# Lynne-Zheng-Linfang/HS-Pose

Hardware: AMD Instinct MI355X
Metric: point-clouds/sec (N=1028) HS-layer fwd+bwd (higher is better)
Workload: dtype f32; 1 GPU; HS stack (FaceRecon backbone -> feat) fwd+bwd, B=16/GPU N=1028 fp32, train-mode BN, random-init weights (BASELINE configs[1] shape); global_batch=16, points=1028, parallelism=dp1, hipgraph=True, split_graph=False, grad_exchange=none

## Files before the change

### hs_pose_amd/csrc/rfconv.hip

```cpp
#include "common.h"
#include "folds.h"
#include <stdlib.h>
#include <atomic>
#include <type_traits>

namespace hsp {

#define RF_THREADS 256

__device__ __forceinline__ void normalise_dirs(float4& d0, float4& d1, float4& d2) {
#define RF_NRM(X)                                                                                    \
    {                                                                                                \
        const float n2 = norm2_chain(d0.X, d1.X, d2.X);                                              \
        const float nr = fmaxf(sqrtf(n2), 1e-12f);                     \
        d0.X = __fdiv_rn(d0.X, nr); d1.X = __fdiv_rn(d1.X, nr); d2.X = __fdiv_rn(d2.X, nr);          \
    }
    RF_NRM(x) RF_NRM(y) RF_NRM(z) RF_NRM(w)
#undef RF_NRM
}
__device__ __forceinline__ void load_dirs_normed(const float* __restrict__ dirs, int SC, int j, float4& d0,
                                                 float4& d1, float4& d2) {
    d0 = *reinterpret_cast<const float4*>(dirs + j);
    d1 = *reinterpret_cast<const float4*>(dirs + SC + j);
    d2 = *reinterpret_cast<const float4*>(dirs + 2 * SC + j);
    normalise_dirs(d0, d1, d2);
}

#ifdef RF_RELU_MAX
#define RF_RELU(X) fmaxf((X), 0.f)
#else
#define RF_RELU(X) __builtin_amdgcn_fmed3f((X), 0.f, 1.f)
#endif

struct PointIter {
    int b0, bstep, i0, istep;
    __device__ __forceinline__ PointIter(int B) {
        const int xcd = blockIdx.x % HSP_NUM_XCD;
        const int local = blockIdx.x / HSP_NUM_XCD;
        const int per_xcd = gridDim.x / HSP_NUM_XCD;
        if (B >= HSP_NUM_XCD) {
            b0 = xcd; bstep = HSP_NUM_XCD; i0 = local; istep = per_xcd;
        } else {
            b0 = xcd % B; bstep = B * HSP_NUM_XCD;
            const int share = xcd / B;
            const int nshare = (HSP_NUM_XCD - b0 + B - 1) / B;
            i0 = local + per_xcd * share; istep = per_xcd * nshare;
        }
    }
};

template <class R3>
__device__ __forceinline__ float rf_dot3(const R3 r, float d0, float d1, float d2) { return dot3_chain(r.x, r.y, r.z, d0, d1, d2); }

template <int NCH>
__device__ __forceinline__ void rf_load_dirs(const float* dirs, int SC, int tid, float4 (&d0)[NCH], float4 (&d1)[NCH],
                                             float4 (&d2)[NCH]) {
    const int nq = SC >> 2;
#pragma unroll
    for (int u = 0; u < NCH; ++u) {
        const int cq = tid + u * RF_THREADS;
        load_dirs_normed(dirs, SC, (cq < nq ? cq : 0) << 2, d0[u], d1[u], d2[u]);
    }
}

template <bool SURFACE, bool WF, typename FT, class Fetch>
__device__ __forceinline__ void rf_group_body(const float4 d0, const float4 d1, const float4 d2, const float4* sR, const int* sIdx,
                                              int k, Fetch fetch, float* smax_j, uint16_t* arg_pj, FT* fwin_pj) {
    float4 best = make_float4(-INFINITY, -INFINITY, -INFINITY, -INFINITY);
    int a0 = 0, a1 = 0, a2 = 0, a3 = 0;
    float4 wf = make_float4(1.f, 1.f, 1.f, 1.f);
#pragma unroll 4
    for (int n = 0; n < k; ++n) {
        const float4 r = sR[n];
        float4 th;
        th.x = RF_RELU(rf_dot3(r, d0.x, d1.x, d2.x));
        th.y = RF_RELU(rf_dot3(r, d0.y, d1.y, d2.y));
        th.z = RF_RELU(rf_dot3(r, d0.z, d1.z, d2.z));
        th.w = RF_RELU(rf_dot3(r, d0.w, d1.w, d2.w));
        if (!SURFACE) {
            const float4 f = fetch(n);
            th.x = mul_rn(th.x, f.x); th.y = mul_rn(th.y, f.y);
            th.z = mul_rn(th.z, f.z); th.w = mul_rn(th.w, f.w);
            if (WF) {
                if (th.x > best.x) wf.x = f.x;
                if (th.y > best.y) wf.y = f.y;
                if (th.z > best.z) wf.z = f.z;
                if (th.w > best.w) wf.w = f.w;
            }
        }
        if (th.x > best.x) { best.x = th.x; a0 = n; }
        if (th.y > best.y) { best.y = th.y; a1 = n; }
        if (th.z > best.z) { best.z = th.z; a2 = n; }
        if (th.w > best.w) { best.w = th.w; a3 = n; }
    }
    *reinterpret_cast<float4*>(smax_j) = best;
    {
        const unsigned lo = (unsigned)sIdx[a0] | ((unsigned)sIdx[a1] << 16);
        const unsigned hi = (unsigned)sIdx[a2] | ((unsigned)sIdx[a3] << 16);
        unsigned* ap = reinterpret_cast<unsigned*>(arg_pj);
        __builtin_nontemporal_store(lo, ap); __builtin_nontemporal_store(hi, ap + 1);
    }
    if (WF) Feat<FT>::st4_nt(fwin_pj, wf);
}

template <bool SURFACE, typename FT>
__device__ __forceinline__ void rf_mean_phase(const float* smax, const FT* fm, FT* out, size_t pt, int S,
                                              int C, float invS_div, int tid) {
    const int fstride = (S + 1) * C;
    for (int c = tid; c < C; c += RF_THREADS) {
        float s = smax[c];
        for (int sp = 1; sp < S; ++sp) s = add_rn(s, smax[sp * C + c]);
        float v = __fdiv_rn(s, invS_div);
        if (!SURFACE) v = add_rn(Feat<FT>::ld(fm + pt * fstride + c), v);
        Feat<FT>::st_nt(out + pt * C + c, v);
    }
}

template <bool SURFACE, int NCH, bool WF, typename FT>
__global__ __launch_bounds__(RF_THREADS) void rf_fwd_kernel(const float* __restrict__ xyz,
                                                            const int32_t* __restrict__ idx,
                                                            const float* __restrict__ dirs,
                                                            const FT* __restrict__ fm, int B, int N, int k,
                                                            int S, int C, FT* __restrict__ out,
                                                            uint16_t* __restrict__ argrow,
                                                            FT* __restrict__ fwin) {
    extern __shared__ __attribute__((aligned(16))) char smem[];
    const int SC = S * C;
    float* smax = reinterpret_cast<float*>(smem);
    float4* sR = reinterpret_cast<float4*>(smax + SC);
    int* sIdx = reinterpret_cast<int*>(sR + k);
    const int tid = threadIdx.x;
    const int nq = SC >> 2;
    const int fstride = (S + 1) * C;
    const float invS_div = (float)S;
    float4 d0[NCH], d1[NCH], d2[NCH];
    rf_load_dirs<NCH>(dirs, SC, tid, d0, d1, d2);
    const PointIter it(B);
    for (int b = it.b0; b < B; b += it.bstep) {
        const float* xb = xyz + (size_t)b * N * 3;
        for (int i = it.i0; i < N; i += it.istep) {
            const size_t pt = (size_t)b * N + i;
            __syncthreads();
            for (int t = tid; t < k; t += RF_THREADS) {
                const int m = idx[pt * k + t];
                sIdx[t] = m;
                const float3 r = unit_dir(xb[i * 3], xb[i * 3 + 1], xb[i * 3 + 2], xb[m * 3], xb[m * 3 + 1], xb[m * 3 + 2]);
                sR[t] = make_float4(r.x, r.y, r.z, 0.f);
            }
            __syncthreads();
#pragma unroll
            for (int u = 0; u < NCH; ++u) {
                const int cq = tid + u * RF_THREADS;
                if (cq < nq) {
                    const int j = cq << 2;
                    const FT* fsup = SURFACE ? nullptr : fm + (size_t)b * N * fstride + C + j;
                    auto fetch = [=](int n) { return Feat<FT>::ld4(fsup + (size_t)sIdx[n] * fstride); };
                    rf_group_body<SURFACE, WF, FT>(d0[u], d1[u], d2[u], sR, sIdx, k, fetch, smax + j, argrow + pt * SC + j,
                                                   WF ? fwin + pt * SC + j : nullptr);
                }
            }
            __syncthreads();
            rf_mean_phase<SURFACE, FT>(smax, fm, out, pt, S, C, invS_div, tid);
        }
    }
}


template <bool SURFACE, int NCH, bool WF, typename FT>
__global__ __launch_bounds__(RF_THREADS) void rf_fwd_pipe_kernel(const float* __restrict__ xyz,
                                                                 const int32_t* __restrict__ idx,
                                                                 const float* __restrict__ dirs,
                                                                 const FT* __restrict__ fm, int B, int N, int k,
                                                                 int S, int C, FT* __restrict__ out,
                                                                 uint16_t* __restrict__ argrow,
                                                                 FT* __restrict__ fwin) {
    extern __shared__ __attribute__((aligned(16))) char smem[];
    const int SC = S * C;
    float* smax2 = reinterpret_cast<float*>(smem);
    float4* sR2 = reinterpret_cast<float4*>(smax2 + 2 * SC);
    int* sIdx2 = reinterpret_cast<int*>(sR2 + 2 * k);
    unsigned* sOff2 = reinterpret_cast<unsigned*>(sIdx2 + 2 * k);
    const int tid = threadIdx.x;
    const int nq = SC >> 2;
    const int fstride = (S + 1) * C;
    const int spare0 = nq - (NCH - 1) * RF_THREADS;
    const float invS_div = (float)S;
    float4 d0[NCH], d1[NCH], d2[NCH];
    rf_load_dirs<NCH>(dirs, SC, tid, d0, d1, d2);
    const PointIter it(B);
    auto dirs_phase = [&](int b, int i, int buf) {
        const int t = tid - spare0;
        if (t >= 0 && t < k) {
            const float* xb = xyz + (size_t)b * N * 3;
            const int m = idx[((size_t)b * N + i) * k + t];
            sIdx2[buf * k + t] = m;
            sOff2[buf * k + t] = (unsigned)m * (unsigned)fstride * (unsigned)sizeof(FT);
            const float3 r = unit_dir(xb[i * 3], xb[i * 3 + 1], xb[i * 3 + 2], xb[m * 3], xb[m * 3 + 1], xb[m * 3 + 2]);
            sR2[buf * k + t] = make_float4(r.x, r.y, r.z, 0.f);
        }
    };
    int b = it.b0, i = it.i0;
    bool have = b < B && i < N;
    if (have) dirs_phase(b, i, 0);
    int cur = 0;
    bool have_prev = false;
    size_t prev_pt = 0;
    while (have) {
        int nb = b, ni = i + it.istep;
        if (ni >= N) { nb = b + it.bstep; ni = it.i0; }
        const bool have_next = nb < B;
        const size_t pt = (size_t)b * N + i;
        __syncthreads();
        if (have_prev) rf_mean_phase<SURFACE, FT>(smax2 + (cur ^ 1) * SC, fm, out, prev_pt, S, C, invS_div, tid);
        if (have_next) dirs_phase(nb, ni, cur ^ 1);
        float* smax = smax2 + cur * SC;
        const float4* sR = sR2 + cur * k;
        const int* sIdx = sIdx2 + cur * k;
        const unsigned* sOff = sOff2 + cur * k;
#pragma unroll
        for (int u = 0; u < NCH; ++u) {
            const int cq = tid + u * RF_THREADS;
            if (cq < nq) {
                const int j = cq << 2;
                const unsigned long long fbase = reinterpret_cast<unsigned long long>(SURFACE ? out : fm + (size_t)b * N * fstride);
                FT* ubase = reinterpret_cast<FT*>(((unsigned long long)__builtin_amdgcn_readfirstlane((unsigned)(fbase >> 32)) << 32) |
                                                  (unsigned)__builtin_amdgcn_readfirstlane((unsigned)fbase));
                const __amdgpu_buffer_rsrc_t frs =
                    __builtin_amdgcn_make_buffer_rsrc(ubase, 0, (int)((size_t)N * fstride * sizeof(FT)), 0x00020000);
                const unsigned voff = (unsigned)(C + j) * (unsigned)sizeof(FT);
                auto fetch = [=](int n) {
                    if constexpr (sizeof(FT) == 4) {
                        const auto v = __builtin_amdgcn_raw_buffer_load_b128(frs, (int)(voff + sOff[n]), 0, 0);
                        return make_float4(__uint_as_float(v[0]), __uint_as_float(v[1]), __uint_as_float(v[2]), __uint_as_float(v[3]));
                    } else {
                        const auto v = __builtin_amdgcn_raw_buffer_load_b64(frs, (int)(voff + sOff[n]), 0, 0);
                        return make_float4(__uint_as_float(v[0] << 16), __uint_as_float(v[0] & 0xffff0000u),
                                           __uint_as_float(v[1] << 16), __uint_as_float(v[1] & 0xffff0000u));
                    }
                };
                rf_group_body<SURFACE, WF, FT>(d0[u], d1[u], d2[u], sR, sIdx, k, fetch, smax + j,
                                               argrow + pt * SC + j, WF ? fwin + pt * SC + j : nullptr);
            }
        }
        have_prev = true; prev_pt = pt;
        cur ^= 1;
        b = nb; i = ni; have = have_next;
    }
    __syncthreads();
    if (have_prev) rf_mean_phase<SURFACE, FT>(smax2 + (cur ^ 1) * SC, fm, out, prev_pt, S, C, invS_div, tid);
}

#define RF_EB 8

template <int NCH>
__global__ __launch_bounds__(RF_THREADS) void rf_conv_bwd_csr_kernel(
    const float* __restrict__ xyz, const float* __restrict__ dirs, const float* __restrict__ fm,
    const uint16_t* __restrict__ argrow, const float* __restrict__ gout, const int32_t* __restrict__ rev_off,
    const int32_t* __restrict__ rev_edge, int B, int N, int k, int S, int C, float* __restrict__ gfm,
    float* __restrict__ ws) {
    extern __shared__ __attribute__((aligned(16))) char smem[];
    const int SC = S * C;
    float* sg = reinterpret_cast<float*>(smem);
    float4* sR = reinterpret_cast<float4*>(sg + RF_EB * C);
    int* sI = reinterpret_cast<int*>(sR + RF_EB);
    const int tid = threadIdx.x;
    const int nq = SC >> 2;
    const int fstride = (S + 1) * C;
    const float invS = 1.0f / (float)S;
    const int cq4 = C >> 2;

    float4 d0[NCH], d1[NCH], d2[NCH], gd0[NCH], gd1[NCH], gd2[NCH];
    rf_load_dirs<NCH>(dirs, SC, tid, d0, d1, d2);
#pragma unroll
    for (int u = 0; u < NCH; ++u) gd0[u] = gd1[u] = gd2[u] = make_float4(0.f, 0.f, 0.f, 0.f);
    const PointIter it(B);
    for (int b = it.b0; b < B; b += it.bstep) {
        const float* xb = xyz + (size_t)b * N * 3;
        const int32_t* offb = rev_off + (size_t)b * (N + 1);
        const int32_t* edgeb = rev_edge + (size_t)b * N * k;
        for (int m = it.i0; m < N; m += it.istep) {
            const size_t pm = (size_t)b * N + m;
            const int o0 = offb[m], o1 = offb[m + 1];
            const float mx = xb[m * 3], my = xb[m * 3 + 1], mz = xb[m * 3 + 2];
            float4 fv[NCH], acc[NCH];
#pragma unroll
            for (int u = 0; u < NCH; ++u) {
                const int cq = tid + u * RF_THREADS;
                acc[u] = make_float4(0.f, 0.f, 0.f, 0.f);
                fv[u] = cq < nq ? *reinterpret_cast<const float4*>(fm + pm * fstride + C + (cq << 2)) : acc[u];
            }
            for (int c = tid; c < C; c += RF_THREADS) gfm[pm * fstride + c] = gout[pm * C + c];
            for (int e0 = o0; e0 < o1; e0 += RF_EB) {
                const int ne = min(RF_EB, o1 - e0);
                __syncthreads();
                if (tid < ne) {
                    const int e = edgeb[e0 + tid];
                    const int i = e / k, n = e - i * k;
                    const float3 r = unit_dir(xb[i * 3], xb[i * 3 + 1], xb[i * 3 + 2], mx, my, mz);
                    sR[tid] = make_float4(r.x, r.y, r.z, __int_as_float(n));
                    sI[tid] = i;
                }
                __syncthreads();
                for (int q = tid; q < ne * cq4; q += RF_THREADS) {
                    const int t = q / cq4, c4 = q - t * cq4;
                    float4 g = *reinterpret_cast<const float4*>(gout + ((size_t)b * N + sI[t]) * C + (c4 << 2));
                    g.x *= invS; g.y *= invS; g.z *= invS; g.w *= invS;
                    *reinterpret_cast<float4*>(sg + t * C + (c4 << 2)) = g;
                }
                __syncthreads();
#pragma unroll
                for (int u = 0; u < NCH; ++u) {
                    const int cq = tid + u * RF_THREADS;
                    if (cq < nq) {
                        const int j = cq << 2;
                        const int c = j % C;
                        ushort4 am[RF_EB];
#pragma unroll
                        for (int t = 0; t < RF_EB; ++t)
                            am[t] = *reinterpret_cast<const ushort4*>(argrow + ((size_t)b * N + sI[t < ne ? t : 0]) * SC + j);
#pragma unroll
                        for (int t = 0; t < RF_EB; ++t) {
                            if (t < ne) {
                                const float4 r = sR[t];
                                const int n = m;
                                const float4 ga = *reinterpret_cast<const float4*>(sg + t * C + c);
#define RF_ONE(X)                                                                                         \
    if (am[t].X == n) {                                                                                   \
        const float z = rf_dot3(r, d0[u].X, d1[u].X, d2[u].X);                                            \
        if (z > 0.f) {                                                                                    \
            acc[u].X += ga.X * z;                                                                         \
            const float w = ga.X * fv[u].X;                                                               \
            gd0[u].X += w * r.x; gd1[u].X += w * r.y; gd2[u].X += w * r.z;                                \
// ... 318 lines not shown
    }
    __syncthreads();
    if (!SURFACE) {
        for (int q = tid; q < (r1 - r0) * G; q += RF_TILE_THREADS) {
            const int m = q / G, g4 = q - m * G;
            const int4 iv = *reinterpret_cast<const int4*>(acc + m * TC + g4 * 4);
            Feat<FT>::st4(gfm + ((size_t)b * N + r0 + m) * fstride + C + j0 + g4 * 4,
                          make_float4((float)iv.x * fx_inv, (float)iv.y * fx_inv, (float)iv.z * fx_inv, (float)iv.w * fx_inv));
        }
        if (D == 0 && j0 < C) {
            for (int q = tid; q < (r1 - r0) * G; q += RF_TILE_THREADS) {
                const int m = q / G, g4 = q - m * G;
                Feat<FT>::st4(gfm + ((size_t)b * N + r0 + m) * fstride + j0 + g4 * 4,
                              Feat<FT>::ld4(gout + ((size_t)b * N + r0 + m) * C + j0 + g4 * 4));
            }
        }
        __syncthreads();
    }
    float* red = reinterpret_cast<float*>(smem);
    float* mine = red + tid * 12;
    mine[0] = g0.x; mine[1] = g0.y; mine[2] = g0.z; mine[3] = g0.w;
    mine[4] = g1.x; mine[5] = g1.y; mine[6] = g1.z; mine[7] = g1.w;
    mine[8] = g2.x; mine[9] = g2.y; mine[10] = g2.z; mine[11] = g2.w;
    __syncthreads();
    if (tid < G * 12) {
        const int gg = tid / 12, w = tid - gg * 12;
        float sacc = 0.f;
        for (int l = 0; l < PL; ++l) sacc += red[(l * G + gg) * 12 + w];
        const int d = w >> 2, e = w & 3;
        gd_part[((size_t)(b * RS + (RS > 1 ? (int)blockIdx.z : 0)) * 3 + d) * SC + j0 + gg * 4 + e] = sacc;
    }
}

__global__ __launch_bounds__(1024) void rf_dirs_reduce_kernel(const float* __restrict__ ws, int nblk, int SC,
                                                              const float* __restrict__ dirs,
                                                              float* __restrict__ out) {
    __shared__ float red[16][3][64];
    dirs_fold_body<1024>(ws, nblk, SC, dirs, out, (int)blockIdx.x, red);
}

static int rf_bwd_grid_max(int SC) {
    long long g = (8ll << 20) / (12ll * SC);
    g &= ~7ll;
    if (g < 8) g = 8;
    if (g > 1024) g = 1024;
    return (int)g;
}

static int rf_bwd_grid(long long points, int SC) {
    const int g = persistent_blocks(points, 4), gm = rf_bwd_grid_max(SC);
    return g < gm ? g : gm;
}

}

using namespace hsp;

static int rf_check(const void* a, const void* b, const void* c, int B, int N, int k, int S, int C) {
    if (!a || !b || !c || B <= 0 || N <= 0 || k <= 0 || S <= 0 || C <= 0) return HSP_ERR_BAD_ARG;
    if (N > 65535 || (C & 3)) return HSP_ERR_UNSUPPORTED;
    return HSP_OK;
}

struct RfFwdPlan { int nch; bool pipe; size_t lds; };
static RfFwdPlan rf_fwd_plan(int k, int S, int C) {
    RfFwdPlan p{0, false, 0};
    if (k <= 0 || S <= 0 || C <= 0 || (C & 3) || (long long)S * C > 4096 || k > 16384) return p;
    const size_t lds = (size_t)(S * C + 5 * k) * 4;
    if (lds > 64 * 1024) return p;
    p.nch = ((S * C >> 2) + RF_THREADS - 1) / RF_THREADS;
    p.lds = lds;
    const int spare0 = (S * C >> 2) - (p.nch - 1) * RF_THREADS;
    const size_t lds_pipe = 2 * (size_t)(S * C + 6 * k) * 4;
    if (spare0 + k <= RF_THREADS && lds_pipe <= 64 * 1024) { p.pipe = true; p.lds = lds_pipe; }
    return p;
}

extern "C" int hsp_rf_fwd_plan(int k, int S, int C, int* pipelined) {
    const RfFwdPlan p = rf_fwd_plan(k, S, C);
    if (pipelined) *pipelined = p.pipe ? 1 : 0;
    return p.nch;
}

template <class F>
static void rf_dispatch_nch(int nch, bool wf, F launch) {
    auto with_wf = [&](auto n) {
        if (wf) launch(n, std::true_type{});
        else launch(n, std::false_type{});
    };
    switch (nch) {
        case 1: with_wf(std::integral_constant<int, 1>{}); break;
        case 2: with_wf(std::integral_constant<int, 2>{}); break;
        case 3: with_wf(std::integral_constant<int, 3>{}); break;
        default: with_wf(std::integral_constant<int, 4>{}); break;
    }
}

template <bool SURFACE, typename FT>
static int rf_fwd(const float* xyz, const int32_t* idx, const float* dirs, const FT* fm, int B, int N, int k,
                  int S, int C, FT* out, uint16_t* argrow, FT* fwin, hspStream_t stream) {
    int rc = rf_check(xyz, idx, dirs, B, N, k, S, C);
    if (rc) return rc;
    if (!out || !argrow || (!SURFACE && !fm)) return HSP_ERR_BAD_ARG;
    const RfFwdPlan plan = rf_fwd_plan(k, S, C);
    if (!plan.nch) return HSP_ERR_UNSUPPORTED;
    const long long npts = (long long)B * N;
    const int grid = persistent_blocks(npts, npts < 2048 ? 4 : npts < 8192 ? 6 : 8);
    rf_dispatch_nch(plan.nch, !SURFACE && fwin, [&](auto nch, auto wf) {
        constexpr int NCH = decltype(nch)::value;
        constexpr bool WF = !SURFACE && decltype(wf)::value;
        auto kern = plan.pipe ? rf_fwd_pipe_kernel<SURFACE, NCH, WF, FT> : rf_fwd_kernel<SURFACE, NCH, WF, FT>;
        hipLaunchKernelGGL(kern, dim3(grid), dim3(RF_THREADS), plan.lds, as_stream(stream), xyz, idx, dirs, fm, B, N, k, S, C, out,
                           argrow, fwin);
    });
    return check_launch();
}

extern "C" int hsp_rf_surface_fwd(const float* xyz, const int32_t* idx, const float* dirs_n, int B, int N, int k,
                                  int S, int K, float* out, uint16_t* argrow, hspStream_t stream) {
    return rf_fwd<true, float>(xyz, idx, dirs_n, nullptr, B, N, k, S, K, out, argrow, nullptr, stream);
}
extern "C" int hsp_rf_surface_fwd_bf16(const float* xyz, const int32_t* idx, const float* dirs_n, int B, int N, int k,
                                       int S, int K, hsp_bf16_t* out, uint16_t* argrow, hspStream_t stream) {
    return rf_fwd<true, bf16_t>(xyz, idx, dirs_n, nullptr, B, N, k, S, K, out, argrow, nullptr, stream);
}

extern "C" int hsp_rf_conv_wants_fwin(int N, int S, int C) {
    (void)N; (void)S; (void)C;
    return 1;
}

extern "C" int hsp_rf_conv_fwd(const float* xyz, const int32_t* idx, const float* dirs_n, const float* fm, int B,
                               int N, int k, int S, int C, float* out, uint16_t* argrow, float* fwin,
                               hspStream_t stream) {
    return rf_fwd<false, float>(xyz, idx, dirs_n, fm, B, N, k, S, C, out, argrow, fwin, stream);
}
extern "C" int hsp_rf_conv_fwd_bf16(const float* xyz, const int32_t* idx, const float* dirs_n, const hsp_bf16_t* fm, int B,
                                    int N, int k, int S, int C, hsp_bf16_t* out, uint16_t* argrow, hsp_bf16_t* fwin,
                                    hspStream_t stream) {
    return rf_fwd<false, bf16_t>(xyz, idx, dirs_n, fm, B, N, k, S, C, out, argrow, fwin, stream);
}
extern "C" int hsp_rf_conv_wants_fwin_bf16(int N, int S, int C) {
    return (size_t)N * (S + 1) * C * sizeof(bf16_t) >= ((size_t)3 << 20) ? 1 : 0;
}

extern "C" size_t hsp_rf_bwd_workspace_bytes(int SC) {
    if (SC <= 0) return 0;
    return (size_t)rf_bwd_grid_max(SC) * 3 * (size_t)SC * sizeof(float);
}

extern "C" int hsp_rf_conv_bwd(const float* xyz, const float* dirs_n, const float* fm, const uint16_t* argrow,
                               const float* grad_out, const int32_t* rev_off, const int32_t* rev_edge, int B, int N,
                               int k, int S, int C, float* grad_fm, float* grad_dirs_n, void* ws, size_t ws_bytes,
                               hspStream_t stream) {
    int rc = rf_check(xyz, dirs_n, fm, B, N, k, S, C);
    if (rc) return rc;
    if (!argrow || !grad_out || !rev_off || !rev_edge || !grad_fm || !grad_dirs_n) return HSP_ERR_BAD_ARG;
    const int SC = S * C;
    if (!ws || ws_bytes < hsp_rf_bwd_workspace_bytes(SC)) return HSP_ERR_WORKSPACE;
    const int nq = SC >> 2;
    const int nch = (nq + RF_THREADS - 1) / RF_THREADS;
    if (nch > 4) return HSP_ERR_UNSUPPORTED;
    hipStream_t st = as_stream(stream);
    const int grid = rf_bwd_grid((long long)B * N, SC);
    const size_t lds = (size_t)(RF_EB * (C + 8)) * 4;
    if (lds > 64 * 1024) return HSP_ERR_UNSUPPORTED;
    float* wsf = reinterpret_cast<float*>(ws);
    rf_dispatch_nch(nch, false, [&](auto n, auto) {
        hipLaunchKernelGGL((rf_conv_bwd_csr_kernel<decltype(n)::value>), dim3(grid), dim3(RF_THREADS), lds, st, xyz, dirs_n, fm, argrow,
                           grad_out, rev_off, rev_edge, B, N, k, S, C, grad_fm, wsf);
    });
    rc = check_launch();
    if (rc) return rc;
    hipLaunchKernelGGL(rf_dirs_reduce_kernel, dim3((SC + 63) / 64), dim3(1024), 0, st, wsf, grid, SC, dirs_n, grad_dirs_n);
    return check_launch();
}

static int pick_tile_cols(int N, int C, bool surface, int B = 0, int SC = 0) {
    if (surface) return (C % 16 == 0) ? 16 : ((C % 8 == 0) ? 8 : 4);
    for (int pass = 0; pass < 2; ++pass)
        for (int tc = 64; tc >= 4; tc >>= 1) {
            if (tc > 16 && (long long)(SC / tc) * B < 2 * HSP_NUM_CU) continue;
            if (C % tc == 0 && ((size_t)N * tc + 3 * (size_t)N) * 4 <= (pass == 0 ? 80u : 156u) * 1024) return tc;
        }
    return 0;
}

extern "C" size_t hsp_rf_bwd_scatter_workspace_bytes(int B, int SC) {
    if (B <= 0 || SC <= 0) return 0;
// ... 167 lines not shown
```

### include/hsp.h

```cpp
#ifndef HSP_H_
#define HSP_H_

#include <stddef.h>
#include <stdint.h>

#ifdef __cplusplus
extern "C" {
#endif

#define HSP_OK 0
#define HSP_ERR_BAD_ARG (-1)
#define HSP_ERR_UNSUPPORTED (-2)
#define HSP_ERR_WORKSPACE (-3)
#define HSP_ERR_LAUNCH (-4)

#define HSP_MAX_K 32

typedef void *hspStream_t;
typedef uint16_t hsp_bf16_t;

int hsp_version(void);
const char *hsp_error_string(int code);
const char *hsp_last_hip_error(void);

size_t hsp_knn_workspace_bytes(int B, int N, int C, int k);
int hsp_knn_f32(const float *x, int B, int N, int C, int k, int drop_first, int32_t *idx,
                void *ws, size_t ws_bytes, hspStream_t stream);
size_t hsp_knn_exact_workspace_bytes(int B, int N, int C, int k, int drop_first);
int hsp_knn_exact_takes(int B, int N, int C, int k, int drop_first);
int hsp_knn_exact_f32(const float *x, int B, int N, int C, int k, int drop_first, int quad_mode, int32_t *idx, void *ws,
                      size_t ws_bytes, int *tie_rows, hspStream_t stream);
size_t hsp_knn_xyz_workspace_bytes(int B, int N);
int hsp_knn_xyz_takes(int B, int N, int k, int drop_first);
int hsp_knn_xyz_f32(const float *xyz, int B, int N, int k, int k2, int drop_first, int32_t *idx, int32_t *idx2, void *ws,
                    size_t ws_bytes, int *tie_rows, hspStream_t stream);
int hsp_geometry_levels_takes(int N0, int N1, int N2, int k1, int kpool, int k2, int drop_first);
int hsp_geometry_levels_f32(const float *xyz, int B, int N0, const int32_t *sel1, int N1, const int32_t *sel2, int N2, int k1,
                            int kpool, int k2, int drop_first, float *v1, float *v2, int32_t *idx1, int32_t *idx1_pool,
                            int32_t *idx2, int32_t *up1, int32_t *up2, hspStream_t stream);
int hsp_geometry_all_takes(int B, int N0, int k0, int kpool0, int N1, int N2, int k1, int kpool, int k2, int drop_first);
size_t hsp_geometry_all_workspace_bytes(int B, int N0);
int hsp_geometry_all_f32(const float *xyz, int B, int N0, int k0, int kpool0, const int32_t *sel1, int N1, const int32_t *sel2, int N2,
                         int k1, int kpool, int k2, int drop_first, int32_t *idx0, int32_t *idx0_pool, float *v1, float *v2,
                         int32_t *idx1, int32_t *idx1_pool, int32_t *idx2, int32_t *up1, int32_t *up2, void *ws, size_t ws_bytes,
                         hspStream_t stream);
int hsp_knn_quadmode_f32(const float *x, int B, int N, int C, int k, int drop_first, int32_t *idx, void *ws, size_t ws_bytes,
                         int quad_mode, hspStream_t stream);
int hsp_quad_outer_f32(const float *x, int B, int N, int C, float *quad, hspStream_t stream);
int hsp_center_cloud_f32(const float *pts, int B, int N, float *centred, float *mean, hspStream_t stream);

int hsp_nn1_f32(const float *tgt, int Nt, const float *src, int Ns, int B, int32_t *idx,
                hspStream_t stream);

int hsp_rf_surface_fwd(const float *xyz, const int32_t *idx, const float *dirs, int B, int N, int k,
                       int S, int K, float *out, uint16_t *argrow, hspStream_t stream);
size_t hsp_rf_bwd_scatter_workspace_bytes(int B, int SC);
int hsp_rf_surface_bwd(const float *xyz, const float *dirs, const uint16_t *argrow, const float *grad_out,
                       int B, int N, int S, int K, float *grad_dirs, void *ws, size_t ws_bytes,
                       hspStream_t stream);

int hsp_rf_conv_wants_fwin(int N, int S, int C);
int hsp_rf_fwd_plan(int k, int S, int C, int *pipelined);
int hsp_rf_conv_fwd(const float *xyz, const int32_t *idx, const float *dirs, const float *fm, int B,
                    int N, int k, int S, int C, float *out, uint16_t *argrow, float *fwin,
                    hspStream_t stream);
int hsp_rf_conv_bwd_scatter(const float *xyz, const float *dirs, const float *fm, const float *fwin,
                            const uint16_t *argrow,
                            const float *grad_out, int B, int N, int S, int C, float *grad_fm,
                            float *grad_dirs, void *ws, size_t ws_bytes, hspStream_t stream);
int hsp_rf_bwd_scatter_plan(int B, int N, int S, int C, int surface, int *row_split);
int hsp_rf_bwd_set_schedule(int legacy);
size_t hsp_rf_bwd_workspace_bytes(int SC);
int hsp_rf_conv_bwd(const float *xyz, const float *dirs, const float *fm, const uint16_t *argrow,
                    const float *grad_out, const int32_t *rev_off, const int32_t *rev_edge, int B, int N,
                    int k, int S, int C, float *grad_fm, float *grad_dirs, void *ws, size_t ws_bytes,
                    hspStream_t stream);

int hsp_rev_build_takes(int n_src);
int hsp_rev_build_edges_in_lds(int n_src, int n_q, int k);
int hsp_rev_build(const int32_t *idx, int B, int Nq, int Nsrc, int k, int kstride, int32_t *rev_off,
                  int32_t *rev_edge, hspStream_t stream);
int hsp_rev_build_multi(int nmaps, const int32_t *const *idx, int B, const int *Nq, const int *Nsrc, const int *k,
                        const int *kstride, int32_t *const *rev_off, int32_t *const *rev_edge, hspStream_t stream);

int hsp_rev_build_sel(const int32_t *idx, const int32_t *qsel, int qsel_stride, int B, int Nidx, int Nq, int Nsrc, int k,
                      int kstride, int32_t *rev_off, int32_t *rev_edge, hspStream_t stream);

int hsp_gather_max_fwd(const float *feat, const int32_t *idx, const int32_t *qsel, int B, int Nsrc,
                       int Nidx, int Nq, int k, int kstride, int C, float *out, uint8_t *argmax,
                       hspStream_t stream);
int hsp_pool_fwd(const float *feat, const float *xyz, const int32_t *idx, const int32_t *qsel, int B, int N, int Nq, int k,
                 int kstride, int C, float *out, uint8_t *argmax, float *xyz_sel, hspStream_t stream);
int hsp_scatter_tile_plan(int B, int Nsrc, int C, int *threads);
int hsp_gather_max_bwd(const float *grad_out, int grad_bcast, const int32_t *idx, const int32_t *qsel,
                       const uint8_t *argmax, int B, int Nsrc, int Nidx, int Nq, int kstride, int C,
                       float *grad_feat, int accumulate ,
                       const float *extra ,
                       hspStream_t stream);
int hsp_gather_max_fwd_sel(const float *feat, const int32_t *idx, const int32_t *qsel, int qsel_stride, int B, int Nsrc,
                           int Nidx, int Nq, int k, int kstride, int C, float *out, uint8_t *argmax, hspStream_t stream);
int hsp_pool_fwd_sel(const float *feat, const float *xyz, const int32_t *idx, const int32_t *qsel, int qsel_stride, int B, int N,
                     int Nq, int k, int kstride, int C, float *out, uint8_t *argmax, float *xyz_sel, hspStream_t stream);
int hsp_gather_max_bwd_sel(const float *grad_out, int grad_bcast, const int32_t *idx, const int32_t *qsel, int qsel_stride,
                           const uint8_t *argmax, int B, int Nsrc, int Nidx, int Nq, int kstride, int C, float *grad_feat,
                           int accumulate, const float *extra, hspStream_t stream);
int hsp_gather_max_bwd_csr(const float *grad_out, int grad_bcast, const uint8_t *argmax, const int32_t *rev_off,
                           const int32_t *rev_edge, int B, int Nsrc, int Nq, int k, int C, float *grad_feat,
                           hspStream_t stream);
int hsp_gather_max_bwd_csr_bf16(const void *grad_out, int grad_bcast, const uint8_t *argmax, const int32_t *rev_off,
                                const int32_t *rev_edge, int B, int Nsrc, int Nq, int k, int C, hsp_bf16_t *grad_feat,
                                hspStream_t stream);

int hsp_points_max_fwd(const float *x, int B, int N, int C, float *out, int32_t *argrow, hspStream_t stream);
int hsp_points_max_bwd(const float *grad_out, const int32_t *argrow, int B, int N, int C, float *grad_x,
                       hspStream_t stream);

size_t hsp_orl_workspace_bytes(int B, int N, int C);
long long hsp_orl_counts_offset(int B, int N, int k, int kstride, int C, size_t ws_bytes);
int hsp_orl_global_fwd(const float *feat, const int32_t *idx, int B, int N, int k, int kstride, int C,
                       float *fg, uint8_t *argmax, void *ws, size_t ws_bytes, hspStream_t stream);
size_t hsp_orl_exact_workspace_bytes(int B, int N, int C);
int hsp_orl_global_exact_f32(const float *feat, const int32_t *idx, int B, int N, int k, int kstride, int C, float *fg,
                             uint8_t *argmax, void *ws, size_t ws_bytes, hspStream_t stream);
int hsp_bn_eval_f32(const float *x, long long R, int C, const float *running_mean, const float *running_var,
                    const float *invstd, const float *weight, const float *bias, float eps, int relu, float *y,
                    hspStream_t stream);
int hsp_exact_layer_takes(int N, int Cin, int C);
int hsp_layer_out_exact_f32(const float *F, int ldf, const float *Wa, int ldwa, const float *fg, int ldfg, const float *Wb,
                            int ldwb, const float *cloud_t, int two_chain, const float *ste, int ldste, const float *xyz3,
                            const float *w3, int relu, int M, int C, int rows_per_cloud, float *out, int ldo,
                            hspStream_t stream);
int hsp_colsum_rows_takes(int C, int elem_bytes);
int hsp_colsum_rows_plan(int B, int N, int C, int elem_bytes, int *rows, int *nchunk, int *row_lanes, int *form);
int hsp_colsum_rows(const float *x, int B, int N, int C, float *out, void *ws, size_t ws_bytes,
                    hspStream_t stream);

int hsp_add_relu_bwd(const float *ga, int lda, const float *gb, int ldb, const float *y, int R, int C, float *out,
                     hspStream_t stream);
int hsp_residual_bias(float *out, const float *f, const float *t, int B, int N, int C, hspStream_t stream);

int hsp_concat_rows(int nseg, const float *const *src, const int32_t *const *idx, const int *width,
                    const int *kind, const int *nsrc, int B, int N, float *out, hspStream_t stream);

int hsp_gather_rows_fwd(const float *feat, const int32_t *idx, int idx_shared, int B, int Nsrc, int Nq,
                        int C, float *out, int out_stride, hspStream_t stream);
// ... 429 lines not shown
```

Before: 10090 point-clouds/sec.

## Add wave-per-point lane kernel for surface receptive-field conv forward

Adds a new forward kernel that maps each wave to one or two points and each lane to a group of four output channels. Normalised directions are cached in LDS once per workgroup, and each wave double-buffers its neighbour-direction list. A cooperative tail path spreads leftover points across waves by support index to balance the final round. A schedule selector routes surface convolutions with C=128 and at least 8192 points to this kernel; the fetch lambda and the group-max are factored into reusable helpers. The aim is to remove the block-wide syncthreads and the separate mean phase of the legacy kernel, at the cost of more LDS use and lower occupancy.

```diff
diff --git a/hs_pose_amd/csrc/rfconv.hip b/hs_pose_amd/csrc/rfconv.hip
--- a/hs_pose_amd/csrc/rfconv.hip
+++ b/hs_pose_amd/csrc/rfconv.hip
@@ -64,8 +64,8 @@
 }
 
 template <bool SURFACE, bool WF, typename FT, class Fetch>
-__device__ __forceinline__ void rf_group_body(const float4 d0, const float4 d1, const float4 d2, const float4* sR, const int* sIdx,
-                                              int k, Fetch fetch, float* smax_j, uint16_t* arg_pj, FT* fwin_pj) {
+__device__ __forceinline__ float4 rf_group_max(const float4 d0, const float4 d1, const float4 d2, const float4* sR, const int* sIdx,
+                                               int k, Fetch fetch, uint16_t* arg_pj, FT* fwin_pj) {
     float4 best = make_float4(-INFINITY, -INFINITY, -INFINITY, -INFINITY);
     int a0 = 0, a1 = 0, a2 = 0, a3 = 0;
     float4 wf = make_float4(1.f, 1.f, 1.f, 1.f);
@@ -93,7 +93,6 @@
         if (th.z > best.z) { best.z = th.z; a2 = n; }
         if (th.w > best.w) { best.w = th.w; a3 = n; }
     }
-    *reinterpret_cast<float4*>(smax_j) = best;
     {
         const unsigned lo = (unsigned)sIdx[a0] | ((unsigned)sIdx[a1] << 16);
         const unsigned hi = (unsigned)sIdx[a2] | ((unsigned)sIdx[a3] << 16);
@@ -101,6 +100,19 @@
         __builtin_nontemporal_store(lo, ap); __builtin_nontemporal_store(hi, ap + 1);
     }
     if (WF) Feat<FT>::st4_nt(fwin_pj, wf);
+    return best;
+}
+template <bool SURFACE, bool WF, typename FT, class Fetch>
+__device__ __forceinline__ void rf_group_body(const float4 d0, const float4 d1, const float4 d2, const float4* sR, const int* sIdx,
+                                              int k, Fetch fetch, float* smax_j, uint16_t* arg_pj, FT* fwin_pj) {
+    *reinterpret_cast<float4*>(smax_j) = rf_group_max<SURFACE, WF, FT>(d0, d1, d2, sR, sIdx, k, fetch, arg_pj, fwin_pj);
+}
+
+__device__ __forceinline__ float rf_mean_add(float sum, float next) { return add_rn(sum, next); }
+template <bool SURFACE>
+__device__ __forceinline__ float rf_mean_finish(float sum, float invS_div, float centre) {
+    const float v = __fdiv_rn(sum, invS_div);
+    return SURFACE ? v : add_rn(centre, v);
 }
 
 template <bool SURFACE, typename FT>
@@ -109,12 +121,35 @@
     const int fstride = (S + 1) * C;
     for (int c = tid; c < C; c += RF_THREADS) {
         float s = smax[c];
-        for (int sp = 1; sp < S; ++sp) s = add_rn(s, smax[sp * C + c]);
-        float v = __fdiv_rn(s, invS_div);
-        if (!SURFACE) v = add_rn(Feat<FT>::ld(fm + pt * fstride + c), v);
+        for (int sp = 1; sp < S; ++sp) s = rf_mean_add(s, smax[sp * C + c]);
+        const float v = rf_mean_finish<SURFACE>(s, invS_div, SURFACE ? 0.f : Feat<FT>::ld(fm + pt * fstride + c));
         Feat<FT>::st_nt(out + pt * C + c, v);
     }
 }
+
+template <typename FT>
+struct RfRowFetch {
+    __amdgpu_buffer_rsrc_t frs;
+    unsigned voff;
+    const unsigned* sOff;
+    __device__ __forceinline__ RfRowFetch(const FT* cloud, int N, int fstride, int col, const unsigned* off) : sOff(off) {
+        const unsigned long long fbase = reinterpret_cast<unsigned long long>(cloud);
+        FT* ubase = reinterpret_cast<FT*>(((unsigned long long)__builtin_amdgcn_readfirstlane((unsigned)(fbase >> 32)) << 32) |
+                                          (unsigned)__builtin_amdgcn_readfirstlane((unsigned)fbase));
+        frs = __builtin_amdgcn_make_buffer_rsrc(ubase, 0, (int)((size_t)N * fstride * sizeof(FT)), 0x00020000);
+        voff = (unsigned)col * (unsigned)sizeof(FT);
+    }
+    __device__ __forceinline__ float4 operator()(int n) const {
+        if constexpr (sizeof(FT) == 4) {
+            const auto v = __builtin_amdgcn_raw_buffer_load_b128(frs, (int)(voff + sOff[n]), 0, 0);
+            return make_float4(__uint_as_float(v[0]), __uint_as_float(v[1]), __uint_as_float(v[2]), __uint_as_float(v[3]));
+        } else {
+            const auto v = __builtin_amdgcn_raw_buffer_load_b64(frs, (int)(voff + sOff[n]), 0, 0);
+            return make_float4(__uint_as_float(v[0] << 16), __uint_as_float(v[0] & 0xffff0000u),
+                               __uint_as_float(v[1] << 16), __uint_as_float(v[1] & 0xffff0000u));
+        }
+    }
+};
 
 template <bool SURFACE, int NCH, bool WF, typename FT>
 __global__ __launch_bounds__(RF_THREADS) void rf_fwd_kernel(const float* __restrict__ xyz,
@@ -222,22 +257,7 @@
             const int cq = tid + u * RF_THREADS;
             if (cq < nq) {
                 const int j = cq << 2;
-                const unsigned long long fbase = reinterpret_cast<unsigned long long>(SURFACE ? out : fm + (size_t)b * N * fstride);
-                FT* ubase = reinterpret_cast<FT*>(((unsigned long long)__builtin_amdgcn_readfirstlane((unsigned)(fbase >> 32)) << 32) |
-                                                  (unsigned)__builtin_amdgcn_readfirstlane((unsigned)fbase));
-                const __amdgpu_buffer_rsrc_t frs =
-                    __builtin_amdgcn_make_buffer_rsrc(ubase, 0, (int)((size_t)N * fstride * sizeof(FT)), 0x00020000);
-                const unsigned voff = (unsigned)(C + j) * (unsigned)sizeof(FT);
-                auto fetch = [=](int n) {
-                    if constexpr (sizeof(FT) == 4) {
-                        const auto v = __builtin_amdgcn_raw_buffer_load_b128(frs, (int)(voff + sOff[n]), 0, 0);
-                        return make_float4(__uint_as_float(v[0]), __uint_as_float(v[1]), __uint_as_float(v[2]), __uint_as_float(v[3]));
-                    } else {
-                        const auto v = __builtin_amdgcn_raw_buffer_load_b64(frs, (int)(voff + sOff[n]), 0, 0);
-                        return make_float4(__uint_as_float(v[0] << 16), __uint_as_float(v[0] & 0xffff0000u),
-                                           __uint_as_float(v[1] << 16), __uint_as_float(v[1] & 0xffff0000u));
-                    }
-                };
+                const RfRowFetch<FT> fetch(SURFACE ? out : fm + (size_t)b * N * fstride, N, fstride, C + j, sOff);
                 rf_group_body<SURFACE, WF, FT>(d0[u], d1[u], d2[u], sR, sIdx, k, fetch, smax + j,
                                                argrow + pt * SC + j, WF ? fwin + pt * SC + j : nullptr);
             }
@@ -248,6 +268,164 @@
     }
     __syncthreads();
     if (have_prev) rf_mean_phase<SURFACE, FT>(smax2 + (cur ^ 1) * SC, fm, out, prev_pt, S, C, invS_div, tid);
+}
+
+#define RF_LANE_WAVES (RF_THREADS / 64)
+template <int Q> struct RfLane {
+    static constexpr int lanes = Q < 64 ? Q : 64;
+    static constexpr int P = 64 / lanes;
+    static constexpr int passes = Q / lanes;
+};
+__host__ __device__ inline size_t rf_lane_lds(int Q, int P, int k, int S) {
+    return (size_t)16 * (3 * S * Q + S * P * Q) + (size_t)RF_LANE_WAVES * 2 * P * k * 24;
+}
+__host__ __device__ inline bool rf_lane_coop(int R, int wgs, int S) {
+    return R > 0 && ((R + wgs - 1) / wgs) * ((S + RF_LANE_WAVES - 1) / RF_LANE_WAVES) < S;
+}
+
+template <bool SURFACE, int Q, bool WF, typename FT>
+__global__ __launch_bounds__(RF_THREADS, 5) void rf_fwd_lane_kernel(const float* __restrict__ xyz,
+                                                                 const int32_t* __restrict__ idx,
+                                                                 const float* __restrict__ dirs,
+                                                                 const FT* __restrict__ fm, int B, int N, int k,
+                                                                 int S, FT* __restrict__ out,
+                                                                 uint16_t* __restrict__ argrow,
+                                                                 FT* __restrict__ fwin) {
+    constexpr int LP = RfLane<Q>::lanes, P = RfLane<Q>::P, NP = RfLane<Q>::passes, C = 4 * Q;
+    extern __shared__ __attribute__((aligned(16))) char smem[];
+    const int SC = S * C;
+    const int fstride = (S + 1) * C;
+    const int tid = threadIdx.x, wave = tid >> 6, lane = tid & 63;
+    const int rk = P * k;
+    float4* sD = reinterpret_cast<float4*>(smem);
+    float4* sMax = sD + 3 * S * Q;
+    float4* sR2 = reinterpret_cast<float4*>(reinterpret_cast<char*>(sMax + S * P * Q) + (size_t)wave * (2 * rk * 24));
+    unsigned* sOff2 = reinterpret_cast<unsigned*>(sR2 + 2 * rk);
+    int* sIdx2 = reinterpret_cast<int*>(sOff2 + 2 * rk);
+    const float invS_div = (float)S;
+    for (int g = tid; g < S * Q; g += RF_THREADS) {
+        float4 d0, d1, d2;
+        load_dirs_normed(dirs, SC, g << 2, d0, d1, d2);
+        const int s = g / Q, cq = g % Q;
+        sD[(3 * s + 0) * Q + cq] = d0; sD[(3 * s + 1) * Q + cq] = d1; sD[(3 * s + 2) * Q + cq] = d2;
+    }
+    __syncthreads();
+
+    const PointIter it(B);
+    const int G = (N + P - 1) / P;
+    const int T = it.b0 < B ? ((B - 1 - it.b0) / it.bstep + 1) * G : 0;
+    const int wslot = it.i0 * RF_LANE_WAVES + wave, nslots = it.istep * RF_LANE_WAVES;
+    const bool coop = rf_lane_coop(T % nslots, it.istep, S);
+    const int lim = coop ? T - T % nslots : T;
+    const int p = lane / LP, cq0 = lane % LP;
+    static_assert(P <= 2, "rec_point");
+    auto rec_point = [&]() { return P == 2 && lane >= k ? 1 : 0; };
+
+    int m_nx = 0;
+    float cx = 0.f, cy = 0.f, cz = 0.f, qx = 0.f, qy = 0.f, qz = 0.f;
+    bool build = false;
+    auto rec_list = [&](int b, int g) {
+        const int rp = rec_point(), i = g * P + rp;
+        build = lane < rk && i < N;
+        if (build) m_nx = idx[((size_t)b * N + i) * k + lane - rp * k];
+    };
+    auto rec_pos = [&](int b, int g) {
+        if (build) {
+            const float* xb = xyz + (size_t)b * N * 3;
+            const int i = g * P + rec_point();
+            cx = xb[i * 3]; cy = xb[i * 3 + 1]; cz = xb[i * 3 + 2];
+            qx = xb[m_nx * 3]; qy = xb[m_nx * 3 + 1]; qz = xb[m_nx * 3 + 2];
+        }
+    };
+    auto rec_publish = [&](int buf) {
+        if (build) {
+            const float3 r = unit_dir(cx, cy, cz, qx, qy, qz);
+            sR2[buf * rk + lane] = make_float4(r.x, r.y, r.z, 0.f);
+            sOff2[buf * rk + lane] = (unsigned)m_nx * (unsigned)fstride * (unsigned)sizeof(FT);
+            sIdx2[buf * rk + lane] = m_nx;
+        }
+        __builtin_amdgcn_fence(__ATOMIC_RELEASE, "wavefront");
+        __builtin_amdgcn_wave_barrier();
+        __builtin_amdgcn_fence(__ATOMIC_ACQUIRE, "wavefront");
+    };
+    auto support_max = [&](int b, size_t pt, int buf, int s, int cq) {
+        const int j = s * C + (cq << 2);
+        RfRowFetch<FT> fetch(SURFACE ? out : fm + (size_t)b * N * fstride, N, fstride, C + j, sOff2 + buf * rk + p * k);
+        return rf_group_max<SURFACE, WF, FT>(sD[(3 * s + 0) * Q + cq], sD[(3 * s + 1) * Q + cq], sD[(3 * s + 2) * Q + cq],
+                                             sR2 + buf * rk + p * k, sIdx2 + buf * rk + p * k, k, fetch, argrow + pt * SC + j,
+                                             WF ? fwin + pt * SC + j : nullptr);
+    };
+    auto store_out = [&](size_t pt, int cq, float4 sum) {
+        float4 ctr = make_float4(0.f, 0.f, 0.f, 0.f);
+        if (!SURFACE) ctr = Feat<FT>::ld4(fm + pt * fstride + (cq << 2));
+        float4 v;
+        v.x = rf_mean_finish<SURFACE>(sum.x, invS_div, ctr.x); v.y = rf_mean_finish<SURFACE>(sum.y, invS_div, ctr.y);
+        v.z = rf_mean_finish<SURFACE>(sum.z, invS_div, ctr.z); v.w = rf_mean_finish<SURFACE>(sum.w, invS_div, ctr.w);
+        Feat<FT>::st4_nt(out + pt * C + (cq << 2), v);
+    };
+
+    int t = wslot, cur = 0;
+    bool have = t < lim;
+    int b = it.b0 + (t / G) * it.bstep, g = t % G;
+    if (have) { rec_list(b, g); rec_pos(b, g); rec_publish(0); }
+    while (have) {
+        t += nslots;
+        const bool have_next = t < lim;
+        const int nb = it.b0 + (t / G) * it.bstep, ng = t % G;
+        if (have_next) rec_list(nb, ng);
+        const int i = g * P + p;
+        const bool live = i < N;
+        const size_t pt = (size_t)b * N + (live ? i : 0);
+#pragma unroll
+        for (int pass = 0; pass < NP; ++pass) {
+            const int cq = cq0 + pass * 64;
+            float4 sum = make_float4(0.f, 0.f, 0.f, 0.f);
+            for (int s = 0; s < S; ++s) {
+                if (live) {
+                    const float4 best = support_max(b, pt, cur, s, cq);
+                    if (s == 0) sum = best;
+                    else {
+                        sum.x = rf_mean_add(sum.x, best.x); sum.y = rf_mean_add(sum.y, best.y);
+                        sum.z = rf_mean_add(sum.z, best.z); sum.w = rf_mean_add(sum.w, best.w);
+                    }
+                }
+            }
+            if (live) store_out(pt, cq, sum);
+        }
+        if (have_next) { rec_pos(nb, ng); rec_publish(cur ^ 1); }
+        cur ^= 1;
+        b = nb; g = ng; have = have_next;
+    }
+
+    if (coop) {
+        for (int ct = lim + it.i0; ct < T; ct += it.istep) {
+            const int cb = it.b0 + (ct / G) * it.bstep, cg = ct % G;
+            rec_list(cb, cg); rec_pos(cb, cg); rec_publish(0);
+            const int i = cg * P + p;
+            if (i < N) {
+                const size_t pt = (size_t)cb * N + i;
+#pragma unroll
+                for (int pass = 0; pass < NP; ++pass) {
+                    const int cq = cq0 + pass * 64;
+                    for (int s = wave; s < S; s += RF_LANE_WAVES) sMax[(s * P + p) * Q + cq] = support_max(cb, pt, 0, s, cq);
+                }
+            }
+            __syncthreads();
+            for (int t = tid; t < P * Q; t += RF_THREADS) {
+                const int tp = t / Q, cq = t % Q;
+                if (cg * P + tp < N) {
+                    float4 sum = sMax[tp * Q + cq];
+                    for (int s = 1; s < S; ++s) {
+                        const float4 best = sMax[(s * P + tp) * Q + cq];
+                        sum.x = rf_mean_add(sum.x, best.x); sum.y = rf_mean_add(sum.y, best.y);
+                        sum.z = rf_mean_add(sum.z, best.z); sum.w = rf_mean_add(sum.w, best.w);
+                    }
+                    store_out((size_t)cb * N + cg * P + tp, cq, sum);
+                }
+            }
+            __syncthreads();
+        }
+    }
 }
 
 #define RF_EB 8
@@ -732,6 +910,53 @@
     return p.nch;
 }
 
+struct RfLanePlan { int q, p; size_t lds; };
+static RfLanePlan rf_lane_plan(int k, int S, int C) {
+    RfLanePlan lp{0, 0, 0};
+    if (!rf_fwd_plan(k, S, C).nch || (C != 128 && C != 256 && C != 512)) return lp;
+    const int q = C / 4, p = q < 64 ? 64 / q : 1;
+    const size_t lds = rf_lane_lds(q, p, k, S);
+    if (p * k > 64 || lds > 64 * 1024) return lp;
+    return RfLanePlan{q, p, lds};
+}
+
+#define RF_LANE_WGS_PER_CU 5
+static int rf_lane_grid(int B, int N, const RfLanePlan& lp) {
+    const long long G = (N + lp.p - 1) / lp.p;
+    const long long T = (B >= HSP_NUM_XCD ? (B + HSP_NUM_XCD - 1) / HSP_NUM_XCD : 1) * G;
+    const long long share = B >= HSP_NUM_XCD ? 1 : HSP_NUM_XCD / B;
+    const long long wmax = (long long)HSP_NUM_CU / HSP_NUM_XCD * RF_LANE_WGS_PER_CU * share;
+    const long long rounds = (T + RF_LANE_WAVES * wmax - 1) / (RF_LANE_WAVES * wmax);
+    long long w = (T + RF_LANE_WAVES * rounds - 1) / (RF_LANE_WAVES * rounds);
+    w = (w + share - 1) / share;
+    return (int)(w < 1 ? 1 : w) * HSP_NUM_XCD;
+}
+
+static std::atomic<int> g_rf_fwd_mode{0};
+#define RF_LANE_MIN_POINTS 8192
+
+static int rf_fwd_schedule(int B, int N, int k, int S, int C, bool surface, int elem_bytes) {
+    (void)elem_bytes;
+    const RfFwdPlan plan = rf_fwd_plan(k, S, C);
+    if (!plan.nch) return HSP_ERR_UNSUPPORTED;
+    const int mode = g_rf_fwd_mode.load();
+    const int legacy = plan.pipe ? 1 : 0;
+    if (mode == 1 || !rf_lane_plan(k, S, C).q) return legacy;
+    if (mode == 2) return 2;
+    return surface && C == 128 && (long long)B * N >= RF_LANE_MIN_POINTS ? 2 : legacy;
+}
+
+extern "C" int hsp_rf_fwd_schedule(int B, int N, int k, int S, int C, int surface, int elem_bytes) {
+    if (B <= 0 || N <= 0 || (elem_bytes != 2 && elem_bytes != 4)) return HSP_ERR_BAD_ARG;
+    if (N > 65535) return HSP_ERR_UNSUPPORTED;
+    return rf_fwd_schedule(B, N, k, S, C, surface != 0, elem_bytes);
+}
+
+extern "C" int hsp_rf_fwd_set_schedule(int mode) {
+    if (mode < 0 || mode > 2) return HSP_ERR_BAD_ARG;
+    return g_rf_fwd_mode.exchange(mode);
+}
+
 template <class F>
 static void rf_dispatch_nch(int nch, bool wf, F launch) {
     auto with_wf = [&](auto n) {
@@ -755,6 +980,25 @@
     const RfFwdPlan plan = rf_fwd_plan(k, S, C);
     if (!plan.nch) return HSP_ERR_UNSUPPORTED;
     const long long npts = (long long)B * N;
+    if (rf_fwd_schedule(B, N, k, S, C, SURFACE, (int)sizeof(FT)) == 2) {
+        const RfLanePlan lp = rf_lane_plan(k, S, C);
+        const int grid = rf_lane_grid(B, N, lp);
+        auto launch = [&](auto q, auto wf) {
+            constexpr bool WF = !SURFACE && decltype(wf)::value;
+            hipLaunchKernelGGL((rf_fwd_lane_kernel<SURFACE, decltype(q)::value, WF, FT>), dim3(grid), dim3(RF_THREADS), lp.lds,
+                               as_stream(stream), xyz, idx, dirs, fm, B, N, k, S, out, argrow, fwin);
+        };
+        auto with_wf = [&](auto q) {
+            if (!SURFACE && fwin) launch(q, std::true_type{});
+            else launch(q, std::false_type{});
+        };
+        switch (lp.q) {
+            case 32: with_wf(std::integral_constant<int, 32>{}); break;
+            case 64: with_wf(std::integral_constant<int, 64>{}); break;
+            default: with_wf(std::integral_constant<int, 128>{}); break;
+        }
+        return check_launch();
+    }
     const int grid = persistent_blocks(npts, npts < 2048 ? 4 : npts < 8192 ? 6 : 8);
     rf_dispatch_nch(plan.nch, !SURFACE && fwin, [&](auto nch, auto wf) {
         constexpr int NCH = decltype(nch)::value;
diff --git a/include/hsp.h b/include/hsp.h
--- a/include/hsp.h
+++ b/include/hsp.h
@@ -61,6 +61,8 @@
 
 int hsp_rf_conv_wants_fwin(int N, int S, int C);
 int hsp_rf_fwd_plan(int k, int S, int C, int *pipelined);
+int hsp_rf_fwd_schedule(int B, int N, int k, int S, int C, int surface, int elem_bytes);
+int hsp_rf_fwd_set_schedule(int mode);
 int hsp_rf_conv_fwd(const float *xyz, const int32_t *idx, const float *dirs, const float *fm, int B,
                     int N, int k, int S, int C, float *out, uint16_t *argrow, float *fwin,
                     hspStream_t stream);
```

Result: no change. 10170 point-clouds/sec (median of 6 runs) (+0.8%).
